# abowman6/CBET_RayTracing_3D

Hardware: AMD Instinct MI355X
Metric: ray-steps/sec, OMEGA 60-beam 256^3 sweep (higher is better)
Workload: dtype f64

## Files before the change

### cbet_raytracing_3d_amd/build.py

```python
import os
import shutil
import subprocess
import sys

PKG = os.path.dirname(os.path.abspath(__file__))
ROOT = os.path.dirname(PKG)
CSRC = os.path.join(PKG, "csrc")
LIB_DIR = os.path.join(PKG, "lib")
LIB_PATH = os.path.join(LIB_DIR, "libcbet_mi355x.so")
SOURCES = ["cbet_kernels.hip", "cbet_trace_window.hip", "cbet_trace_exit.hip", "cbet_trace_path.hip", "cbet_grid_kernels.hip", "cbet_lpi.hip", "cbet_sph_modes.hip",
           "cbet_target.hip", "cbet_mesh.hip", "cbet_mesh_deposit.hip", "cbet_params.cpp", "cbet_context.cpp", "cbet_tables_abi.cpp", "cbet_trace_abi.cpp", "cbet_gain_abi.cpp",
           "cbet_host.cpp", "cbet_output.cpp", "cbet_sph_host.cpp", "cbet_target_host.cpp", "cbet_mesh_host.cpp", "cbet_mesh_deposit_host.cpp",
           "cbet_exchange_host.cpp", "cbet_lpi_host.cpp"]
HEADERS = [os.path.join(CSRC, "cbet_device.h"), os.path.join(CSRC, "cbet_host_internal.h"), os.path.join(CSRC, "cbet_relocate.h"), os.path.join(CSRC, "cbet_trace_common.h"), os.path.join(CSRC, "cbet_trace_diag.h"), os.path.join(CSRC, "cbet_hd.h"), os.path.join(CSRC, "cbet_node_model.h"), os.path.join(CSRC, "cbet_node_kernel.h"), os.path.join(CSRC, "cbet_target_model.h"), os.path.join(CSRC, "cbet_mesh_model.h"), os.path.join(CSRC, "cbet_state_model.h"), os.path.join(CSRC, "cbet_mesh_deposit_model.h"), os.path.join(CSRC, "cbet_gain_model.h"), os.path.join(CSRC, "cbet_lpi_model.h"), os.path.join(ROOT, "include", "cbet_mi355x.h"),
           os.path.join(ROOT, "include", "cbet_omega_beams.h")]

FLAGS = ["-O3", "-std=c++17", "--offload-arch=gfx950", "-ffp-contract=off", "-fPIC", "-shared",
         "-Wall", "-Wextra", "-Wno-unused-result", "-mllvm", "-structurizecfg-skip-uniform-regions=true"]


def hipcc():
    exe = shutil.which("hipcc") or "/opt/rocm/bin/hipcc"
    if not os.path.exists(exe):
        raise RuntimeError("hipcc not found (need ROCm to build the gfx950 library)")
    return exe


def is_stale():
    if not os.path.exists(LIB_PATH):
        return True
    built = os.path.getmtime(LIB_PATH)
    deps = [os.path.join(CSRC, s) for s in SOURCES] + HEADERS + [os.path.abspath(__file__),
                                                                os.path.join(ROOT, "tools", "cbet_gpu.cpp"),
                                                                os.path.join(ROOT, "tools", "cbet_reference_shaped.cpp"),
                                                                os.path.join(ROOT, "include", "cbet_reference_api.hpp")]
    return any(os.path.getmtime(d) > built for d in deps)


def build(force=False, verbose=False, extra_flags=()):
    if not force and not is_stale():
        return LIB_PATH
    os.makedirs(LIB_DIR, exist_ok=True)
    cmd = [hipcc()] + FLAGS + list(extra_flags) + [
        "-I", os.path.join(ROOT, "include"), "-I", CSRC,
        "-o", LIB_PATH] + [os.path.join(CSRC, s) for s in SOURCES] + ["-lrccl"]
    if verbose:
        print(" ".join(cmd), flush=True)
    run = subprocess.run(cmd, stderr=subprocess.PIPE, text=True)
    sys.stderr.write(run.stderr)
    if run.returncode != 0 and "structurizecfg-skip-uniform-regions" in run.stderr:
        print("build: this hipcc does not know -structurizecfg-skip-uniform-regions; building without it", flush=True)
        k = cmd.index("-structurizecfg-skip-uniform-regions=true")
        subprocess.check_call(cmd[:k - 1] + cmd[k + 1:])
    elif run.returncode != 0:
        raise subprocess.CalledProcessError(run.returncode, cmd)
    build_cli(verbose)
    build_ref_shaped(verbose)
    return LIB_PATH


CLI_PATH = os.path.join(PKG, "lib", "cbet-gpu")


def build_cli(verbose=False):
    cmd = ["g++", "-O2", "-std=c++17", "-I", os.path.join(ROOT, "include"),
           os.path.join(ROOT, "tools", "cbet_gpu.cpp"), "-o", CLI_PATH,
           "-L", LIB_DIR, "-lcbet_mi355x", "-Wl,-rpath,$ORIGIN", "-Wl,-rpath-link," + "/opt/rocm/lib"]
    if verbose:
        print(" ".join(cmd), flush=True)
    subprocess.check_call(cmd)
    return CLI_PATH


REF_SHAPED_PATH = os.path.join(PKG, "lib", "cbet-ref-shaped")


def build_ref_shaped(verbose=False):
    cmd = [hipcc(), "-O2", "-std=c++17", "-I", os.path.join(ROOT, "include"),
           os.path.join(ROOT, "tools", "cbet_reference_shaped.cpp"), "-o", REF_SHAPED_PATH,
           "-L", LIB_DIR, "-lcbet_mi355x", "-Wl,-rpath,$ORIGIN"]
    if verbose:
        print(" ".join(cmd), flush=True)
    subprocess.check_call(cmd)
    return REF_SHAPED_PATH


def build_variant(name, extra_flags=(), verbose=False):
    out_dir = os.path.join(ROOT, "build_alt")
    os.makedirs(out_dir, exist_ok=True)
    out = os.path.join(out_dir, "libcbet_%s.so" % name)
    cmd = [hipcc()] + FLAGS + list(extra_flags) + ["-I", os.path.join(ROOT, "include"), "-I", CSRC, "-o", out] + \
        [os.path.join(CSRC, s) for s in SOURCES] + ["-lrccl"]
    if verbose:
        print(" ".join(cmd), flush=True)
    subprocess.check_call(cmd)
    return out


if __name__ == "__main__":
    if len(sys.argv) > 2 and sys.argv[1] == "--variant":
        print(build_variant(sys.argv[2], sys.argv[3:], verbose=True))
    else:
        print(build(force="--force" in sys.argv, verbose=True))
```

### cbet_raytracing_3d_amd/csrc/cbet_trace_window.hip

```cpp
#include <hip/hip_runtime.h>

#include <cstddef>
#include <type_traits>

#if defined(__HIP_DEVICE_COMPILE__) && !defined(__gfx950__)
#error "cbet_trace_window.hip is written for gfx950 (CDNA4) only"
#endif

#include "cbet_trace_common.h"
#include "cbet_trace_diag.h"

namespace cbet {
namespace {

#define CBET_BALLOT(cond) __builtin_amdgcn_ballot_w64(cond)
#define CBET_LANES(mask) __builtin_amdgcn_inverse_ballot_w64(mask)
#define CBET_USUAL(cond) __builtin_expect(!!(cond), 1)
#define CBET_RARE(cond) __builtin_expect(!!(cond), 0)
#define CBET_SELDOM(cond) __builtin_expect_with_probability(!!(cond), 0, 0.9)

template <int WX_, int WY_, int WZ_, bool PAD, bool XORSW = false>
struct Tile {
    static constexpr int WX = WX_, WY = WY_, WZ = WZ_;
    static constexpr int XM = WX - 1, YM = WY - 1, ZM = WZ - 1;
    static constexpr bool ROT = PAD && WZ == 16;
    static constexpr int YS = (PAD && !ROT) ? WZ + 1 : WZ;
    static constexpr int XS = (PAD && !ROT) ? WY * YS + 4 : WY * WZ;
    static constexpr bool XOR = ROT && XORSW;
    static __device__ __forceinline__ int zr(int tx, int ty, int tz)
    {
        return XOR ? (tz ^ ((tx & 3) << 2) ^ (ty << 1)) : (ROT ? ((tz + 7 * tx + 3 * ty) & ZM) : tz);
    }
    static_assert(!XOR || (WX == 8 && WY == 8 && WZ == 16), "the swizzle terms are written for the 8 x 8 x 16 box");
    static __device__ __forceinline__ int xterm(int tx) { return __mul24(tx, XS * 8 + 32) & ~0x80; }
    static __device__ __forceinline__ int yterm(int ty) { return __mul24(ty, YS * 8 + 16); }
    static constexpr int N = WX * XS;
    static constexpr int SX = WX - 2, SY = WY - 2, SZ = WZ - 2;
    static constexpr bool BRICK = WZ == 16 && WY == 8;
    static constexpr int DT = WX * WY * WZ;
    static __device__ __forceinline__ int slot_d(int tx, int ty, int tz) { return (tx * WY + ty) * WZ + tz; }
};

struct Origin {
    int x, y, z;
};

template <int M>
__device__ __forceinline__ int abs_in(int o, int r) { return o + ((r - o) & M); }

template <int C>
struct Corner {
    static constexpr int index = C;
    template <class V> static __device__ __forceinline__ V x(V v0, V v1) { return (C & 1) ? v1 : v0; }
    template <class V> static __device__ __forceinline__ V z(V v0, V v1) { return (C & 2) ? v1 : v0; }
    template <class V> static __device__ __forceinline__ V y(V v0, V v1) { return (C & 4) ? v1 : v0; }
};
template <class F>
__device__ __forceinline__ void each_corner(F f)
{
    f(Corner<0>{}); f(Corner<1>{}); f(Corner<2>{}); f(Corner<3>{}); f(Corner<4>{}); f(Corner<5>{}); f(Corner<6>{}); f(Corner<7>{});
}

struct WaveCounters {
    int n_atomics = 0;
    int n_miss = 0;
    unsigned steps_miss = 0;
    unsigned slabs_bsteps = 0;
    int pend = 0;
    [[no_unique_address]] WaveDiag dg;
};

template <bool W32>
struct Grid {
    double *p;
};
template <bool W32>
__device__ __forceinline__ void grid_add(const TraceArgs &a, Grid<W32> g, int node, double v)
{
    if constexpr (W32) global_add(a, reinterpret_cast<double *>(reinterpret_cast<char *>(g.p) + ((unsigned)node * 8u)), v);
    else global_add(a, &g.p[node], v);
}
template <bool W32>
__device__ __forceinline__ void grid_add_far(const TraceArgs &a, Grid<W32> g, long index, double v) { global_add(a, &g.p[index], v); }

template <class G>
__device__ __forceinline__ void write_back(const TraceArgs &a, double *tile, int slot, G edep, int node, double v, WaveCounters &wc)
{
    wc.pend += (CBET_BALLOT(v != 0.0) != 0ull) ? 1 : 0;
    if (v != 0.0) {
        tile[slot] = 0.0;
        ++wc.n_atomics;
        grid_add(a, edep, node, v);
    }
}
template <class G>
__device__ __forceinline__ void write_back_far(const TraceArgs &a, double *tile, int slot, G edep, long index, double v, WaveCounters &wc)
{
    wc.pend += (CBET_BALLOT(v != 0.0) != 0ull) ? 1 : 0;
    if (v != 0.0) {
        grid_add_far(a, edep, index, v);
        tile[slot] = 0.0;
        ++wc.n_atomics;
    }
}

template <class F>
__device__ __forceinline__ void miss_add8(unsigned long long hbm_m, WaveCounters &wc, F add8)
{
    if (CBET_RARE(hbm_m != 0ull)) {
        wc.pend += 8;
        if (CBET_LANES(hbm_m)) add8();
    }
}

template <class T, int AX, int COUNT, class G>
__device__ __forceinline__ void retire_planes(const TraceArgs &a, double *tile, const Origin &o, int coord, int step,
                                              int lane, G edep, int sXh, int sYh, WaveCounters &wc)
{
    constexpr int WO = AX == 0 ? T::WY : T::WX, OM = WO - 1;
    constexpr int IT = (WO * T::WZ + kWave - 1) / kWave;
    constexpr int RS = kWave / T::WZ;
    static_assert(IT == 1 || (IT == 2 && 2 * RS == WO), "a plane is one entry per lane, or two in the halves of the other axis");
    static_assert(!T::XOR || IT == 1 || (RS == 4 && T::YS == 16 && T::XS == 128), "the second entry's slot is written for the 8 x 8 x 16 box");
    constexpr int SLOT_X = AX == 0 ? (RS * T::YS) ^ ((2 * RS) & T::ZM) : RS * T::XS;
    const int r0 = lane / T::WZ, r1 = lane & T::ZM, k = abs_in<T::ZM>(o.z, r1);
    const int d0 = (r0 - (AX == 0 ? o.y : o.x)) & OM, dnode = ((d0 & RS) ? -RS : RS) * (AX == 0 ? sYh : sXh);
    const bool in_plane = !(WO * T::WZ < kWave) || lane < WO * T::WZ;
    double v[COUNT * IT];
    int slot[COUNT * IT], node[COUNT * IT];
#pragma unroll
    for (int pl = 0; pl < COUNT; ++pl) {
        const int c = coord + pl * step;
        const int fixed = c & (AX == 0 ? T::XM : T::YM);
#pragma unroll
        for (int e = 0; e < IT; ++e) {
            const int q = pl * IT + e, re = r0 + e * RS;
            if (e == 1 && T::XOR) {
                slot[q] = slot[q - 1] ^ SLOT_X;
                node[q] = node[q - 1] + dnode;
            } else if (AX == 0) {
                slot[q] = fixed * T::XS + re * T::YS + T::zr(fixed, re, r1);
                node[q] = c * sXh + __mul24(abs_in<T::YM>(o.y, re), sYh) + k;
            } else {
                slot[q] = re * T::XS + fixed * T::YS + T::zr(re, fixed, r1);
                node[q] = __mul24(abs_in<T::XM>(o.x, re), sXh) + c * sYh + k;
            }
            const bool ok = in_plane && CBET_AUDIT(a, (unsigned)slot[q] < (unsigned)T::N);
            v[q] = ok ? tile[slot[q]] : 0.0;
        }
    }
#pragma unroll
    for (int q = 0; q < COUNT * IT; ++q) write_back(a, tile, slot[q], edep, node[q], v[q], wc);
}

template <class T, int AX, int NC, class G>
__device__ __forceinline__ void retire_plane(const TraceArgs &a, double *tile, const Origin &o, int coord, int lane,
                                             G edep, int sXh, int sYh, WaveCounters &wc, int coff, long gstride)
{
    constexpr int WO = AX == 0 ? T::WY : T::WX;
    constexpr int IT = (WO * T::WZ + kWave - 1) / kWave;
    const int fixed = coord & (AX == 0 ? T::XM : T::YM);
#pragma unroll
    for (int e = 0; e < IT; ++e) {
        const int idx = e * kWave + lane;
        const bool in_plane = !(WO * T::WZ < kWave) || idx < WO * T::WZ;
        const int r0 = idx / T::WZ, r1 = idx & T::ZM;
        int slot, node, slot_d;
        const int k = abs_in<T::ZM>(o.z, r1);
        if (AX == 0) {
            slot = fixed * T::XS + r0 * T::YS + T::zr(fixed, r0, r1);
            slot_d = T::slot_d(fixed, r0, r1);
            node = coord * sXh + __mul24(abs_in<T::YM>(o.y, r0), sYh) + k;
        } else {
            slot = r0 * T::XS + fixed * T::YS + T::zr(r0, fixed, r1);
            slot_d = T::slot_d(r0, fixed, r1);
            node = __mul24(abs_in<T::XM>(o.x, r0), sXh) + coord * sYh + k;
        }
        const bool ok = in_plane && CBET_AUDIT(a, (unsigned)slot < (unsigned)T::N);
        const double v = ok ? tile[slot] : 0.0;
        if (NC > 1) {
#pragma unroll
            for (int q = 1; q < NC; ++q) {
                const int sq = coff + (q - 1) * T::DT + slot_d;
                write_back_far(a, tile, sq, edep, q * gstride + node, ok ? tile[sq] : 0.0, wc);
            }
        }
        write_back(a, tile, slot, edep, node, v, wc);
    }
}

template <class T, int NC, class G>
__device__ __forceinline__ void retire_zplane(const TraceArgs &a, double *tile, const Origin &o, int coord, int lane,
                                              G edep, int sXh, int sYh, WaveCounters &wc, int coff, long gstride)
{
    static_assert(T::WX * T::WY <= kWave, "one z-plane entry per lane");
    const int r0 = lane / T::WY, r1 = lane & T::YM, fixed = coord & T::ZM;
    const int slot = r0 * T::XS + r1 * T::YS + T::zr(r0, r1, fixed);
    const int node = __mul24(abs_in<T::XM>(o.x, r0), sXh) + __mul24(abs_in<T::YM>(o.y, r1), sYh) + coord;
    const bool ok = (!(T::WX * T::WY < kWave) || lane < T::WX * T::WY) && CBET_AUDIT(a, (unsigned)slot < (unsigned)T::N);
    const double v = ok ? tile[slot] : 0.0;
    if (NC > 1) {
        const int slot_d = T::slot_d(r0, r1, fixed);
#pragma unroll
        for (int q = 1; q < NC; ++q) {
            const int sq = coff + (q - 1) * T::DT + slot_d;
            write_back_far(a, tile, sq, edep, q * gstride + node, ok ? tile[sq] : 0.0, wc);
        }
    }
    write_back(a, tile, slot, edep, node, v, wc);
}

template <class T, class G>
__device__ __forceinline__ void retire_zbrick(const TraceArgs &a, double *tile, const Origin &o, int zb, int lane,
                                              G edep, int sXh, int sYh, WaveCounters &wc)
{
    static_assert(T::WY == 8 && T::WZ == 16, "a brick is 8 rows of 8 planes per tile x index");
    const int ty = lane >> 3, kz = lane & 7;
    const int tz = (zb + kz) & T::ZM;
    const int base_node = __mul24(abs_in<T::YM>(o.y, ty), sYh) + zb + kz;
    constexpr int ROUND = 4;
#pragma unroll
    for (int t0 = 0; t0 < T::WX; t0 += ROUND) {
        double v[ROUND];
        int slot[ROUND];
#pragma unroll
        for (int q = 0; q < ROUND; ++q) {
            slot[q] = (t0 + q) * T::XS + ty * T::YS + T::zr(t0 + q, ty, tz);
            v[q] = CBET_AUDIT(a, (unsigned)slot[q] < (unsigned)T::N) ? tile[slot[q]] : 0.0;
        }
#pragma unroll
        for (int q = 0; q < ROUND; ++q) write_back(a, tile, slot[q], edep, abs_in<T::XM>(o.x, t0 + q) * sXh + base_node, v[q], wc);
    }
}

template <class T, int NC, class G>
__device__ __forceinline__ void flush_box(const TraceArgs &a, double *tile, const Origin &o, int lane, G edep,
                                          int sXh, int sYh, WaveCounters &wc, int coff, long gstride)
{
    for (int t = 0; t < T::WX; ++t)
        retire_plane<T, 0, NC>(a, tile, o, o.x + t, lane, edep, sXh, sYh, wc, coff, gstride);
}

__device__ __forceinline__ int follow_plane_axis(int r, unsigned long long mm, int S)
{
    const unsigned long long edge = __builtin_amdgcn_ballot_w64((unsigned)(r - 1) >= (unsigned)(S - 1)) & mm;
    if (CBET_USUAL(edge == 0ull)) return 0;
    const unsigned long long hi = __builtin_amdgcn_ballot_w64(r >= S) & edge;
    const bool at_hi = hi != 0ull, at_lo = hi != edge;
    if (at_hi == at_lo) return 0;
    if (at_hi) {
        if ((__builtin_amdgcn_ballot_w64(r <= 1) & mm) != 0ull) return (__builtin_amdgcn_ballot_w64(r > S) & mm) != 0ull ? 1 : 0;
        return (S >= 6 && (__builtin_amdgcn_ballot_w64(r <= 2) & mm) == 0ull) ? 2 : 1;
    }
    if ((__builtin_amdgcn_ballot_w64(r >= S - 1) & mm) != 0ull) return (__builtin_amdgcn_ballot_w64(r < 0) & mm) != 0ull ? -1 : 0;
    return (S >= 6 && (__builtin_amdgcn_ballot_w64(r >= S - 2) & mm) == 0ull) ? -2 : -1;
}

__device__ __forceinline__ int follow_brick_axis(int r, unsigned long long mm)
{
    if ((__builtin_amdgcn_ballot_w64((unsigned)r > 14u) & mm) == 0ull) return 0;
    const bool below = (__builtin_amdgcn_ballot_w64(r < 0) & mm) != 0ull, above = (__builtin_amdgcn_ballot_w64(r > 14) & mm) != 0ull;
    const bool needs_lo = (__builtin_amdgcn_ballot_w64(r <= 7) & mm) != 0ull, needs_hi = (__builtin_amdgcn_ballot_w64(r >= 7) & mm) != 0ull;
    return (below && !needs_hi) ? -1 : ((above && !needs_lo) ? 1 : 0);
}

template <class T, int NC, class G>
__device__ __forceinline__ bool follow_box(const TraceArgs &a, double *tile, Origin &o, unsigned long long mm, int lx,
                                           int ly, int lz, int lane, G edep, int sXh, int sYh, WaveCounters &wc,
                                           int coff, long gstride)
{
    auto leave = [&](auto axis, int d, int lo, int hi) {
        constexpr int AX = decltype(axis)::value;
        const int first = d < 0 ? hi : lo, step = d < 0 ? -1 : 1, n = d < 0 ? -d : d;
        if constexpr (NC == 1) {
            if (n == 2) retire_planes<T, AX, 2>(a, tile, o, first, step, lane, edep, sXh, sYh, wc);
            else retire_planes<T, AX, 1>(a, tile, o, first, step, lane, edep, sXh, sYh, wc);
        } else {
            for (int q = 0; q < n; ++q) retire_plane<T, AX, NC>(a, tile, o, first + q * step, lane, edep, sXh, sYh, wc, coff, gstride);
        }
    };
    const int dx = follow_plane_axis(lx - o.x, mm, T::SX);
    const int dy = follow_plane_axis(ly - o.y, mm, T::SY);
    if (dx != 0) { wc.dg.retire_begin(); leave(std::integral_constant<int, 0>{}, dx, o.x, o.x + T::WX - 1); wc.dg.retire_end(); }
    o.x += dx;
    if (dy != 0) { wc.dg.retire_begin(); leave(std::integral_constant<int, 1>{}, dy, o.y, o.y + T::WY - 1); wc.dg.retire_end(); }
    o.y += dy;
    int dz;
    if constexpr (T::BRICK) {
        dz = 8 * follow_brick_axis(lz - o.z, mm);
        if (dz != 0) { wc.dg.retire_begin(); retire_zbrick<T>(a, tile, o, dz < 0 ? o.z + 8 : o.z, lane, edep, sXh, sYh, wc); wc.dg.retire_end(); }
    } else {
        dz = follow_plane_axis(lz - o.z, mm, T::SZ);
        if (dz != 0)
            retire_zplane<T, NC>(a, tile, o, dz < 0 ? o.z + T::WZ - 1 : o.z, lane, edep, sXh, sYh, wc, coff, gstride);
        for (int q = 1; q < (dz < 0 ? -dz : dz); ++q)
            retire_zplane<T, NC>(a, tile, o, dz < 0 ? o.z + T::WZ - 1 - q : o.z + q, lane, edep, sXh, sYh, wc, coff, gstride);
    }
    o.z += dz;
    const bool moved = (dx | dy | dz) != 0;
    wc.slabs_bsteps += moved ? (1u << 16) : 0u;
    return moved;
}

template <class T>
__device__ __forceinline__ bool holds(const Origin &o, int lx, int ly, int lz)
{
    return (unsigned)(lx - o.x) <= (unsigned)T::SX && (unsigned)(ly - o.y) <= (unsigned)T::SY &&
           (unsigned)(lz - o.z) <= (unsigned)T::SZ;
}

template <class T>
__device__ __forceinline__ int box_near_axes(const Origin &o, int nx, int ny, int nz)
{
    const int lo = kRelocateDeep + 1;
    const unsigned tx = (unsigned)((o.x - lo) | (nx - 3 - T::SX - o.x)), ty = (unsigned)((o.y - lo) | (ny - 3 - T::SY - o.y)),
                   tz = (unsigned)((o.z - lo) | (nz - 3 - T::SZ - o.z));
    return (int)((tx >> 31) | ((ty >> 31) << 1) | ((tz >> 31) << 2));
}

typedef double dbl2 __attribute__((ext_vector_type(2)));

template <bool WIDE>
__device__ __forceinline__ void record_issue(const StepRecord *base, unsigned cell, dbl2 &kxy, dbl2 &kzk)
{
    if constexpr (WIDE) {
        const char *p = reinterpret_cast<const char *>(base) + ((unsigned long long)cell << 5);
        asm volatile("global_load_dwordx4 %0, %2, off\n\tglobal_load_dwordx4 %1, %2, off offset:16\n\t; CBET_RECORD_ISSUE %0 %1"
                     : "=&v"(kxy), "=&v"(kzk)
                     : "v"(p)
                     : "memory");
    } else {
        const unsigned off = cell << 5;
        asm volatile("s_nop 4\n\tglobal_load_dwordx4 %0, %2, %3\n\tglobal_load_dwordx4 %1, %2, %3 offset:16\n\t; CBET_RECORD_ISSUE %0 %1"
                     : "=&v"(kxy), "=&v"(kzk)
                     : "v"(off), "s"(base)
                     : "memory");
    }
}

__device__ __forceinline__ void record_wait(dbl2 &kxy, dbl2 &kzk, int pend)
{
    asm volatile("; CBET_RECORD_WAIT %0 %1\n\t"
                 "s_cmp_eq_u32 %2, 0\n\t"
                 "s_cbranch_scc1 .Lrw_0_%=\n\t"
                 "s_cmp_ge_u32 %2, 8\n\t"
                 "s_cbranch_scc1 .Lrw_8_%=\n\t"
                 "s_cmp_ge_u32 %2, 4\n\t"
                 "s_cbranch_scc1 .Lrw_4_%=\n\t"
                 "s_cmp_ge_u32 %2, 2\n\t"
                 "s_cbranch_scc1 .Lrw_2_%=\n\t"
                 "s_waitcnt vmcnt(1)\n\t"
                 "s_branch .Lrw_end_%=\n"
                 ".Lrw_2_%=:\n\t"
                 "s_waitcnt vmcnt(2)\n\t"
                 "s_branch .Lrw_end_%=\n"
                 ".Lrw_4_%=:\n\t"
                 "s_waitcnt vmcnt(4)\n\t"
                 "s_branch .Lrw_end_%=\n"
                 ".Lrw_8_%=:\n\t"
                 "s_waitcnt vmcnt(8)\n\t"
                 "s_branch .Lrw_end_%=\n"
                 ".Lrw_0_%=:\n\t"
                 "s_waitcnt vmcnt(0)\n"
                 ".Lrw_end_%=:"
                 : "+v"(kxy), "+v"(kzk)
                 : "s"(pend)
                 : "memory", "scc");
}

__device__ __forceinline__ void record_wait_all(dbl2 &kxy, dbl2 &kzk)
{
    asm volatile("; CBET_RECORD_WAIT %0 %1\n\ts_waitcnt vmcnt(0)" : "+v"(kxy), "+v"(kzk) : : "memory");
}

__device__ __forceinline__ void exit_planes_load(dbl2 &bx, dbl2 &by, dbl2 &bz)
{
    const void *args = (const void *)__builtin_amdgcn_kernarg_segment_ptr();
    asm volatile("s_load_dwordx4 %0, %3, %4\n\ts_load_dwordx4 %1, %3, %5\n\ts_load_dwordx4 %2, %3, %6\n\ts_waitcnt lgkmcnt(0)"
                 : "=&s"(bx), "=&s"(by), "=&s"(bz)
                 : "s"(args), "i"(offsetof(TraceArgs, exit_planes)), "i"(offsetof(TraceArgs, exit_planes) + 16),
                   "i"(offsetof(TraceArgs, exit_planes) + 32));
}

__device__ __forceinline__ int add3(int a, int b, int c)
{
    int r;
    asm("v_add3_u32 %0, %1, %2, %3" : "=v"(r) : "v"(a), "v"(b), "v"(c));
    return r;
}

__device__ __forceinline__ int xad1(int f, int c)
{
    int r;
    asm("v_xad_u32 %0, %1, 1, %2" : "=v"(r) : "v"(f), "v"(c));
    return r;
}

__device__ __forceinline__ double max_abs3(double a, double b, double c)
{
    double r;
    asm("v_max_f64 %0, |%1|, |%2|" : "=v"(r) : "v"(a), "v"(b));
    asm("v_max_f64 %0, %1, |%2|" : "=v"(r) : "v"(r), "v"(c));
    return r;
}

__device__ __forceinline__ void commit(int &var, int value)
{
    asm volatile("s_mov_b32 %0, %1" : "+s"(var) : "s"(__builtin_amdgcn_readfirstlane(value)));
}
__device__ __forceinline__ void commit(unsigned long long &var, unsigned long long value)
{
    asm volatile("s_mov_b64 %0, %1" : "+s"(var) : "s"(value));
}
__device__ __forceinline__ void commit_v(int &var, int value) { asm volatile("v_mov_b32 %0, %1" : "+v"(var) : "v"(value)); }

__device__ __forceinline__ void cell_step(int &c, unsigned long long up, unsigned long long dn)
{
    asm("s_nop 1\n\tv_addc_co_u32_e64 %0, vcc, 0, %0, %1\n\tv_subbrev_co_u32_e64 %0, vcc, 0, %0, %2" : "+v"(c) : "s"(up), "s"(dn) : "vcc");
}
__device__ __forceinline__ void cell_step3(int &ci, int &cj, int &ck, unsigned long long upx, unsigned long long dnx,
                                           unsigned long long upy, unsigned long long dny, unsigned long long upz,
                                           unsigned long long dnz)
{
    asm("s_nop 1\n\t"
        "v_addc_co_u32_e64 %0, vcc, 0, %0, %3\n\tv_addc_co_u32_e64 %1, vcc, 0, %1, %5\n\tv_addc_co_u32_e64 %2, vcc, 0, %2, %7\n\t"
        "v_subbrev_co_u32_e64 %0, vcc, 0, %0, %4\n\tv_subbrev_co_u32_e64 %1, vcc, 0, %1, %6\n\tv_subbrev_co_u32_e64 %2, vcc, 0, %2, %8"
        : "+v"(ci), "+v"(cj), "+v"(ck)
        : "s"(upx), "s"(dnx), "s"(upy), "s"(dny), "s"(upz), "s"(dnz)
        : "vcc");
}

__device__ __forceinline__ int mad24(int a, int b, int c)
{
    int r;
    asm("s_nop 1\n\tv_mad_i32_i24 %0, %1, %2, %3" : "=v"(r) : "v"(a), "s"(b), "v"(c));
    return r;
}


#ifdef CBET_DEBUG_BOUNDS
constexpr bool kAudited = true;
#else
constexpr bool kAudited = false;
#endif
constexpr double kNearTol = 0.5001;
constexpr double kFarJump = 1.4998;

template <int WZ, bool GENERIC, int CBET, bool STATS>
__global__ void __launch_bounds__(kWave, (CBET == 4) ? 1 : 4) k_trace_window(const TraceArgs a)
{
    using T = Tile<8, 8, WZ, true, CBET == 0>;
    using TB = Tile<4, 8, 8, false>;
    constexpr bool IDX64 = GENERIC;
    constexpr int NC = (CBET == 4) ? 4 : 1;
    constexpr bool ACC = (CBET == 0);
    constexpr bool PIPE = ACC;
    constexpr int NSLOT = T::N + TB::N;
    constexpr int NLDS = NSLOT + (NC - 1) * T::DT;
    __shared__ double s_val[NLDS];
    const int lane = threadIdx.x;

    int beam, patch;
    if (!work_item(a, blockIdx.x, beam, patch)) return;
    const Grid<!IDX64> edep{a.edep + (long)(beam - a.grid_beam0) * a.grid_stride};
    const bool absorb = GENERIC ? (a.absorption == 1) : true;

    Ray s = {};
    int li;
    const bool launched = launch_lane(a, beam, patch, lane, s, li);
    unsigned long long live = __ballot(launched);
    if (live == 0ull) return;
    const int tot_rays = __popcll(live);

    const int nx = a.nx, ny = a.ny, nz = a.nz;
    const int sYh = a.sYh, sXh = a.sXh;
    unsigned cell = launched ? (unsigned)((s.ci * ny + s.cj) * nz + s.ck) : 0u;
    double fcx = (double)s.ci, fcy = (double)s.cj, fcz = (double)s.ck;
    int tot_steps = 0;
    WaveCounters wc;

    double *const tileA = s_val, *const tileB = s_val + T::N;
    Origin oA{0, 0, 0}, oB{0, 0, 0};
    unsigned long long hbm = 0ull;
    int b_active = 0;
    {
        const int src = ((live >> 27) & 1ull) ? 27 : (__ffsll((long long)live) - 1);
        for (int z = lane; z < NLDS; z += kWave) s_val[z] = 0.0;
        oA.x = __builtin_amdgcn_readlane(s.ci, src) + 1 - T::WX / 2;
        oA.y = __builtin_amdgcn_readlane(s.cj, src) + 1 - T::WY / 2;
        oA.z = __builtin_amdgcn_readlane(s.ck, src) + 1 - 4;
        if (T::BRICK) oA.z &= ~7;
        __syncthreads();
    }
    int near = 7;
    wc.dg.begin();

    dbl2 rec_kxy, rec_kzk;
    const StepRecord *rec_base = a.steprec;
    asm volatile("" : "+s"(rec_base));
    double dt = a.dt;
    auto gather_record = [&]() {
        unsigned c = CBET_LANES(live) ? cell : 0u;
        asm("" : "+v"(c));
#ifdef CBET_DEBUG_BOUNDS
        if (!(c < a.audit_nodes)) { audit_fail(a); c = 0u; }
#endif
        record_issue<IDX64>(rec_base, c, rec_kxy, rec_kzk);
        wc.pend = 0;
    };
    auto await_record = [&]() {
        wc.dg.wait_begin();
        if (CBET == 0 && !kAudited) record_wait(rec_kxy, rec_kzk, wc.pend);
        else record_wait_all(rec_kxy, rec_kzk);
        wc.dg.wait_end();
    };
    gather_record();
    await_record();
    const double *const gk = CBET && a.gain ? a.gain + (long)(beam - a.grid_beam0) * a.hsize : nullptr;
    double gained = 0.0;

    const bool flx = (lane & 1) != 0, fly = (lane & 2) != 0, flz = (lane & 8) != 0;
    const int pfx = flx ? 1 : 0, pfy = fly ? 1 : 0, pfz = flz ? 1 : 0;

    double q0 = 0.0, q1 = 0.0, q2 = 0.0, q3 = 0.0;

    int slow = 7;
    double Fx0 = 0, Fx1 = 0, Fy0 = 0, Fy1 = 0, Fz0 = 0, Fz1 = 0;
    int X0 = 0, X1 = 0, Y0 = 0, Y1 = 0, Z0 = 0, Z1 = 0;
    double inc = 0.0;
    int tile_off = 0;
    unsigned long long miss_m = 0ull;
    int own_slot = 0, own_node = 0;
    auto lds_add8 = [&](const double *w) {
        auto add = [&](int byte, double v) {
            if (CBET_AUDIT(a, (unsigned)byte < (unsigned)NSLOT * 8u))
                __hip_atomic_fetch_add(static_cast<double *>(__builtin_assume_aligned(reinterpret_cast<char *>(s_val) + byte, 8)),
                                       v, __ATOMIC_RELAXED, __HIP_MEMORY_SCOPE_WORKGROUP);
        };
        if constexpr (T::XOR) {
            int ax0, ax1, by0, by1, cz0, cz1;
            if (CBET_USUAL(b_active == 0)) {
                ax0 = T::xterm(X0 & T::XM); ax1 = T::xterm(X1 & T::XM);
                by0 = T::yterm(Y0 & T::YM); by1 = T::yterm(Y1 & T::YM);
                cz0 = (Z0 & T::ZM) << 3; cz1 = (Z1 & T::ZM) << 3;
            } else {
                const bool toB = tile_off != 0;
                const int xm = toB ? TB::XM : T::XM, zm = toB ? TB::ZM : T::ZM;
                const int xmul = toB ? TB::XS * 8 : T::XS * 8 + 32, ymul = toB ? TB::YS * 8 : T::YS * 8 + 16;
                const int keep = toB ? ~0 : ~0x80, off8 = tile_off * 8;
                static_assert(TB::YM == T::YM, "one y mask for both boxes");
                ax0 = (__mul24(X0 & xm, xmul) & keep) | off8; ax1 = (__mul24(X1 & xm, xmul) & keep) | off8;
                by0 = __mul24(Y0 & T::YM, ymul); by1 = __mul24(Y1 & T::YM, ymul);
                cz0 = (Z0 & zm) << 3; cz1 = (Z1 & zm) << 3;
            }
            auto at = [](int ax, int by, int cz) { return (int)__builtin_amdgcn_bitop3_b32(ax, by, cz, 0x96); };
            each_corner([=](auto c) { add(at(c.x(ax0, ax1), c.y(by0, by1), c.z(cz0, cz1)), w[c.index]); });
        } else {
            auto add8 = [&](int xm, int ym, int zm, int xs, int ys, int off, int rot) {
                const int xa = X0 & xm, xb = X1 & xm, ya = Y0 & ym, yb = Y1 & ym;
                const int x0 = __mul24(xa, xs * 8) + off * 8, x1 = __mul24(xb, xs * 8) + off * 8;
                const int y0 = __mul24(ya, ys * 8), y1 = __mul24(yb, ys * 8);
                const int ra = 7 * xa * rot, rb = 7 * xb * rot, sa = 3 * ya * rot, sb = 3 * yb * rot;
                auto zb = [&](int z, int r) { return ((z + r) & zm) * 8; };
                if constexpr (T::ROT) {
                    const int xy00 = x0 | y0, xy10 = x1 | y0, xy01 = x0 | y1, xy11 = x1 | y1, zm8 = zm * 8;
                    auto at = [&](int xy, int z, int r) { return (((z + r) * 8) & zm8) | xy; };
                    each_corner([&](auto c) {
                        add(at(c.y(c.x(xy00, xy10), c.x(xy01, xy11)), c.z(Z0, Z1), c.x(ra, rb) + c.y(sa, sb)), w[c.index]);
                    });
                } else {
                    each_corner([&](auto c) {
                        add(add3(c.x(x0, x1), c.y(y0, y1), zb(c.z(Z0, Z1), c.x(ra, rb) + c.y(sa, sb))), w[c.index]);
                    });
                }
            };
            if (b_active == 0) {
                add8(T::XM, T::YM, T::ZM, T::XS, T::YS, 0, T::ROT ? 1 : 0);
            } else {
                const bool toB = tile_off != 0;
                add8(toB ? TB::XM : T::XM, toB ? TB::YM : T::YM, toB ? TB::ZM : T::ZM, toB ? TB::XS : T::XS,
                     toB ? TB::YS : T::YS, tile_off, (T::ROT && !toB) ? 1 : 0);
            }
        }
    };
    auto hbm_add8 = [&](const double *w) {
        const int nX0 = __mul24(X0, sXh), nX1 = __mul24(X1, sXh), nY0 = __mul24(Y0, sYh), nY1 = __mul24(Y1, sYh);
        each_corner([&](auto c) { grid_add(a, edep, c.x(nX0, nX1) + c.y(nY0, nY1) + c.z(Z0, Z1), w[c.index]); });
        wc.n_atomics += 8;
    };

    auto deposit_step = [&](unsigned long long lds_m, unsigned long long hbm_m) {
        const double zi0 = Fz0 * inc, zi1 = Fz1 * inc;
        const double zy00 = zi0 * Fy0, zy10 = zi1 * Fy0, zy01 = zi0 * Fy1, zy11 = zi1 * Fy1;
        double wgt[8];
        wgt[0] = zy00 * Fx0;
        wgt[1] = zy00 * Fx1;
        wgt[2] = zy10 * Fx0;
        wgt[3] = zy10 * Fx1;
        wgt[4] = zy01 * Fx0;
        wgt[5] = zy01 * Fx1;
        wgt[6] = zy11 * Fx0;
        wgt[7] = zy11 * Fx1;
        if (CBET_LANES(lds_m)) lds_add8(wgt);
        miss_add8(hbm_m, wc, [&]() {
            hbm_add8(wgt);
            ++wc.n_miss;
        });
        if (CBET == 4) {
            const bool inbox = CBET_LANES(lds_m);
            if (inbox && tile_off == 0) {
                if (CBET_AUDIT(a, (unsigned)(own_slot + 2 * T::DT) < (unsigned)NLDS)) {
                    __hip_atomic_fetch_add(&s_val[own_slot], q1, __ATOMIC_RELAXED, __HIP_MEMORY_SCOPE_WORKGROUP);
                    __hip_atomic_fetch_add(&s_val[own_slot + T::DT], q2, __ATOMIC_RELAXED, __HIP_MEMORY_SCOPE_WORKGROUP);
                    __hip_atomic_fetch_add(&s_val[own_slot + 2 * T::DT], q3, __ATOMIC_RELAXED, __HIP_MEMORY_SCOPE_WORKGROUP);
                }
            } else if (inbox || CBET_LANES(hbm_m)) {
                grid_add_far(a, edep, a.comp_stride + own_node, q1);
                grid_add_far(a, edep, 2 * a.comp_stride + own_node, q2);
                grid_add_far(a, edep, 3 * a.comp_stride + own_node, q3);
                wc.n_atomics += 3;
            }
        }
    };

    double S[8] = {0, 0, 0, 0, 0, 0, 0, 0};
    unsigned long long restart_m = 0ull;
    bool p_odd = true;
    auto accumulate = [&]() {
        const double zi0 = Fz0 * inc, zi1 = Fz1 * inc;
        const double zy00 = zi0 * Fy0, zy10 = zi1 * Fy0, zy01 = zi0 * Fy1, zy11 = zi1 * Fy1;
        const double k = CBET_LANES(restart_m) ? 0.0 : 1.0;
        auto add = [&](double &sum, double w) { asm("v_fma_f64 %0, %0, %1, %2" : "+v"(sum) : "v"(k), "v"(w)); };
        add(S[0], zy00 * Fx0);
        add(S[1], zy00 * Fx1);
        add(S[2], zy10 * Fx0);
        add(S[3], zy10 * Fx1);
        add(S[4], zy01 * Fx0);
        add(S[5], zy01 * Fx1);
        add(S[6], zy11 * Fx0);
        add(S[7], zy11 * Fx1);
    };
    auto flush_sums = [&](unsigned long long lds_m, unsigned long long hbm_m) {
        if (CBET_LANES(lds_m)) lds_add8(S);
        miss_add8(hbm_m, wc, [&]() { hbm_add8(S); });
    };

    auto step_tail = [&](int &tt) {
    asm volatile("" : "+v"(Fx0), "+v"(Fx1), "+v"(Fy0), "+v"(Fy1), "+v"(Fz0), "+v"(Fz1));
    await_record();
    if (absorb) {
        inc = rec_kzk.y * s.uray;
        s.uray -= inc;
    } else {
        inc = s.uray;
    }
    if (CBET >= 2) inc = q0;
    if constexpr (ACC && !PIPE) accumulate();
    unsigned long long died = CBET_BALLOT(s.uray <= s.ustop);
    const int faces = slow | near;
    if (CBET_RARE(faces != 0)) {
        dbl2 bx, by, bz;
        exit_planes_load(bx, by, bz);
        if (faces & 1) died |= CBET_BALLOT(s.px < bx.x) | CBET_BALLOT(s.px > bx.y);
        if (faces & 2) died |= CBET_BALLOT(s.py < by.x) | CBET_BALLOT(s.py > by.y);
        if (faces & 4) died |= CBET_BALLOT(s.pz < bz.x) | CBET_BALLOT(s.pz > bz.y);
    }
    died &= live;
    if (CBET_SELDOM(died != 0ull)) {
        asm volatile("");
        commit(tot_steps, tot_steps + __popcll(died) * (tt + 1));
        if constexpr (PIPE) {
            accumulate();
            asm volatile("v_mov_b64 %0, 0" : "+v"(inc));
            commit(restart_m, 0ull);
        }
        if constexpr (ACC) flush_sums(died & ~miss_m, died & miss_m);
        else deposit_step(died & ~miss_m, died & miss_m);
        commit(live, live & ~died);
        commit(hbm, hbm & live);
        commit(miss_m, miss_m & live);
        if (live == 0ull) commit(tt, a.nt - 1);
    }
    __builtin_amdgcn_wave_barrier();
    };

    for (int tt = 0; tt < a.nt; ++tt) {
        if constexpr (STATS || WaveDiag::kCountsWaveSteps) wc.steps_miss += 1u << 16;
        wc.dg.step_begin(near);
        s.vx -= rec_kxy.x;
        s.vy -= rec_kxy.y;
        s.vz -= rec_kzk.x;
        asm volatile("" : "+s"(dt));
        s.px += s.vx * dt;
        s.py += s.vy * dt;
        s.pz += s.vz * dt;
        const double fx = (s.px - a.xmin) * a.inv_dx;
        const double fy = (s.py - a.ymin) * a.inv_dy;
        const double fz = (s.pz - a.zmin) * a.inv_dz;
        const double g0x = fx - fcx, g0y = fy - fcy, g0z = fz - fcz;
        const unsigned long long upx = CBET_BALLOT(g0x >= kNearTol), dnx = CBET_BALLOT(g0x < kNearTol - 1.0),
                                 upy = CBET_BALLOT(g0y >= kNearTol), dny = CBET_BALLOT(g0y < kNearTol - 1.0),
                                 upz = CBET_BALLOT(g0z >= kNearTol), dnz = CBET_BALLOT(g0z < kNearTol - 1.0);
        slow = ((CBET_BALLOT(!(max_abs3(g0x, g0y, g0z) < kFarJump)) & live) != 0ull) ? 7 : near;
        if (CBET_USUAL(slow == 0)) {
            cell_step3(s.ci, s.cj, s.ck, upx, dnx, upy, dny, upz, dnz);
        } else {
            if (slow & 1) s.ci = relocate_closed(s.ci, fx, nx);
            else cell_step(s.ci, upx, dnx);
            if (slow & 2) s.cj = relocate_closed(s.cj, fy, ny);
            else cell_step(s.cj, upy, dny);
            if (slow & 4) s.ck = relocate_closed(s.ck, fz, nz);
            else cell_step(s.ck, upz, dnz);
        }
        const unsigned new_cell = (unsigned)mad24(mad24(s.ci, ny, s.cj), nz, s.ck);
        unsigned long long moved_m = 0ull;
        if constexpr (ACC) moved_m = CBET_BALLOT(new_cell != cell);
        cell = new_cell;
        gather_record();
        wc.dg.chain_end();
        asm volatile("" : "+v"(s.ci), "+v"(s.cj), "+v"(s.ck), "+v"(inc));
        fcx = (double)s.ci;
        fcy = (double)s.cj;
        fcz = (double)s.ck;
        if constexpr (!ACC) deposit_step(live & ~miss_m, miss_m);
        if constexpr (PIPE) accumulate();
        const double ox = (fx - fcx) - 0.5, oy = (fy - fcy) - 0.5, oz = (fz - fcz) - 0.5;
        const bool ngx = ox < 0, ngy = oy < 0, ngz = oz < 0;
        const bool all_negative = (live & ~(CBET_BALLOT(ngx) & CBET_BALLOT(ngy) & CBET_BALLOT(ngz))) == 0ull;
        if constexpr (ACC) {
            const unsigned long long fl_m = (all_negative && !p_odd) ? (live & moved_m) : live;
            if (CBET_USUAL(fl_m != 0ull)) {
                if (CBET_USUAL(miss_m == 0ull)) flush_sums(fl_m, 0ull);
                else flush_sums(fl_m & ~miss_m, fl_m & miss_m);
            }
            restart_m = fl_m;
            p_odd = !all_negative;
        }
        factor_pair(ox, pfx, Fx0, Fx1);
        factor_pair(oy, pfy, Fy0, Fy1);
        factor_pair(oz, pfz, Fz0, Fz1);
        int rx, ry, rz;
        if (CBET_USUAL(all_negative)) {
            rx = s.ci - oA.x;
            ry = s.cj - oA.y;
            rz = s.ck - oA.z;
            asm("" : "+v"(rx), "+v"(ry), "+v"(rz));
            X0 = xad1(pfx, s.ci); X1 = s.ci + pfx;
            Y0 = xad1(pfy, s.cj); Y1 = s.cj + pfy;
            Z0 = xad1(pfz, s.ck); Z1 = s.ck + pfz;
        } else {
            const int lx = s.ci + 1 - (ngx ? 1 : 0);
            const int ly = s.cj + 1 - (ngy ? 1 : 0);
            const int lz = s.ck + 1 - (ngz ? 1 : 0);
            rx = lx - oA.x;
            ry = ly - oA.y;
            rz = lz - oA.z;
            const bool hx = ngx != flx, hy = ngy != fly, hz = ngz != flz;
            X0 = lx + (hx ? 1 : 0); X1 = lx + (hx ? 0 : 1);
            Y0 = ly + (hy ? 1 : 0); Y1 = ly + (hy ? 0 : 1);
            Z0 = lz + (hz ? 1 : 0); Z1 = lz + (hz ? 0 : 1);
        }
        if (CBET && CBET_LANES(live)) {
            double ds = 0.0;
            if (gk || CBET >= 2) ds = sqrt_speed(__builtin_fma(s.vz, s.vz, __builtin_fma(s.vy, s.vy, s.vx * s.vx))) * a.dt;
            double u_eff = s.uray;
            if (gk) {
                const double x = gain_exponent<IDX64>(a, gk, X0, X1, Y0, Y1, Z0, Z1, Fx0, Fx1, Fy0, Fy1, Fz0, Fz1, sXh, sYh, ds);
                const double phi = gain_phi(x, (CBET_BALLOT(!(fabs(x) < kPhiSmallBelow)) & live) == 0ull);
                const double dg = s.uray * (x * phi);
                u_eff = s.uray * phi;
                gained += dg;
                s.uray = s.uray + dg;
            }
            if (CBET == 2) q0 = u_eff * ds;
            if (CBET == 4) {
                q0 = u_eff * ds;
                q1 = u_eff * (s.vx * a.dt);
                q2 = u_eff * (s.vy * a.dt);
                q3 = u_eff * (s.vz * a.dt);
                const int hi = s.ci + 1, hj = s.cj + 1, hk = s.ck + 1;
                own_slot = T::slot_d(hi & T::XM, hj & T::YM, hk & T::ZM) + NSLOT;
                own_node = __mul24(hi, sXh) + __mul24(hj, sYh) + hk;
            }
        }
        const unsigned long long memA = live & ~hbm;
        unsigned long long out_core = memA & ~(CBET_BALLOT((unsigned)rx <= (unsigned)T::SX) & CBET_BALLOT((unsigned)ry <= (unsigned)T::SY) &
                                               CBET_BALLOT((unsigned)rz <= (unsigned)T::SZ));
        if (CBET_RARE(b_active != 0)) {
            asm volatile("");
            if constexpr (STATS) wc.slabs_bsteps += 1u;
            const int abx = oA.x - oB.x, aby = oA.y - oB.y, abz = oA.z - oB.z;
            out_core |= hbm & ~(CBET_BALLOT((unsigned)(rx + abx) <= (unsigned)TB::SX) &
                                CBET_BALLOT((unsigned)(ry + aby) <= (unsigned)TB::SY) &
                                CBET_BALLOT((unsigned)(rz + abz) <= (unsigned)TB::SZ));
            tile_off = CBET_LANES(hbm) ? T::N : 0;
        }
        out_core |= miss_m;
        if (CBET_RARE(out_core != 0ull)) {
            wc.dg.arm_begin();
            const bool alive = CBET_LANES(live);
            int lx = rx + oA.x, ly = ry + oA.y, lz = rz + oA.z;
            asm volatile("" : "+v"(lx), "+v"(ly), "+v"(lz));
            Origin nA = oA, nB = oB;
            unsigned long long n_hbm = hbm, n_miss = 0ull;
            int n_bact = b_active, n_near, n_toff = tile_off;
            follow_box<T, NC>(a, tileA, nA, memA, lx, ly, lz, lane, edep, sXh, sYh, wc, NSLOT, a.comp_stride);
            const unsigned long long lost_mask =
                memA & ~(CBET_BALLOT((unsigned)(lx - nA.x) <= (unsigned)T::SX) & CBET_BALLOT((unsigned)(ly - nA.y) <= (unsigned)T::SY) &
                         CBET_BALLOT((unsigned)(lz - nA.z) <= (unsigned)T::SZ));
            if (CBET_USUAL(lost_mask == 0ull && n_bact == 0)) {
                n_near = box_near_axes<T>(nA, nx, ny, nz);
            } else {
                bool homeB = CBET_LANES(hbm);
                const bool inA = alive && holds<T>(nA, lx, ly, lz);
                const bool lost = alive && !homeB && !inA;
                if (n_bact != 0) {
                    follow_box<TB, 1>(a, tileB, nB, hbm, lx, ly, lz, lane, edep, sXh, sYh, wc, 0, 0);
                } else if (lost_mask != 0ull) {
                    const int src = __ffsll((long long)lost_mask) - 1;
                    const int sx = __builtin_amdgcn_readlane(lx, src), sy = __builtin_amdgcn_readlane(ly, src),
                              sz = __builtin_amdgcn_readlane(lz, src);
                    nB.x = sx - (TB::WX / 2 - 1);
                    nB.y = sy - (TB::WY / 2 - 1);
                    nB.z = sz - TB::SZ / 2;
                    n_bact = 1;
                }
                const bool inB = alive && holds<TB>(nB, lx, ly, lz);
                homeB = homeB || (lost && inB);
                if (alive && homeB && !inB && inA) homeB = false;
                n_hbm = CBET_BALLOT(alive && homeB);
                if (n_hbm == 0ull) {
                    __builtin_amdgcn_wave_barrier();
                    flush_box<TB, 1>(a, tileB, nB, lane, edep, sXh, sYh, wc, 0, 0);
                    n_bact = 0;
                }
                __builtin_amdgcn_wave_barrier();
                const bool useB = alive && homeB && inB;
                n_toff = useB ? T::N : 0;
                n_miss = live & ~CBET_BALLOT(useB || (alive && !homeB && inA));
                if constexpr (STATS) {
                    if (n_miss != 0ull) wc.steps_miss += 1u;
                    if (ACC && CBET_LANES(n_miss)) ++wc.n_miss;
                }
                n_near = n_miss != 0ull ? 7 : (box_near_axes<T>(nA, nx, ny, nz) | (n_bact == 0 ? 0 : box_near_axes<TB>(nB, nx, ny, nz)));
            }
            commit(oA.x, nA.x); commit(oA.y, nA.y); commit(oA.z, nA.z);
            commit(oB.x, nB.x); commit(oB.y, nB.y); commit(oB.z, nB.z);
            commit(hbm, n_hbm); commit(miss_m, n_miss);
            commit(b_active, n_bact); commit(near, n_near);
            commit_v(tile_off, n_toff);
            wc.pend = __builtin_amdgcn_readfirstlane(wc.pend);
            wc.dg.arm_end();
        } else if (CBET_RARE(near != 0)) {
            commit(near, box_near_axes<T>(oA, nx, ny, nz) | (b_active == 0 ? 0 : box_near_axes<TB>(oB, nx, ny, nz)));
        }
        step_tail(tt);
    }
    tot_steps += __popcll(live) * a.nt;

    if constexpr (PIPE) accumulate();
    if constexpr (ACC) flush_sums(live & ~miss_m, live & miss_m);
    else deposit_step(live & ~miss_m, live & miss_m);
    __syncthreads();
    flush_box<T, NC>(a, tileA, oA, lane, edep, sXh, sYh, wc, NSLOT, a.comp_stride);
    if (b_active != 0) flush_box<TB, 1>(a, tileB, oB, lane, edep, sXh, sYh, wc, 0, 0);

    if (CBET && a.beam_gain) {
        double t = gained;
#pragma unroll
        for (int off = 32; off > 0; off >>= 1) t += __shfl_xor(t, off, kWave);
        if (lane == 0 && t != 0.0) atomicAdd(&a.beam_gain[beam], t);
    }
    if (wc.dg.report(a, lane, tot_steps, tot_rays, wc.steps_miss >> 16)) return;
    if constexpr (STATS) {
        const int tot_at = wave_sum(wc.n_atomics), tot_miss = wave_sum(wc.n_miss);
        if (lane == 0) {
            atomicAdd(&a.counters[kCntGlobalAtomics], (unsigned long long)tot_at);
            atomicAdd(&a.counters[kCntEvictions], (unsigned long long)tot_miss);
            atomicAdd(&a.counters[kCntWaveSteps], (unsigned long long)(wc.steps_miss >> 16));
            atomicAdd(&a.counters[kCntWaveStepsMiss], (unsigned long long)(wc.steps_miss & 0xFFFFu));
            atomicAdd(&a.counters[kCntWaveStepsWide], (unsigned long long)(wc.slabs_bsteps & 0xFFFFu));
            atomicAdd(&a.counters[kCntSlabsRetired], (unsigned long long)(wc.slabs_bsteps >> 16));
        }
    }
    if (lane == 0) {
        atomicAdd(&a.counters[kCntSteps], (unsigned long long)tot_steps);
        atomicAdd(&a.counters[kCntRays], (unsigned long long)tot_rays);
    }
}

}

hipError_t launch_trace_window(const TraceArgs &a, bool force_idx64, hipStream_t stream)
{
    const long waves = a.item_count;
    if (waves <= 0) return hipSuccess;
    const dim3 grid((unsigned)waves), block(kWave);
    const unsigned long long grid_bytes = 8ull * (unsigned long long)a.sXh * (unsigned long long)(a.nx + 2);
    const bool generic = force_idx64 || (a.gain && 8ull * (unsigned long long)a.hsize >= (1ull << 32)) || a.absorption != 1 ||
                         grid_bytes >= (1ull << 32) ||
                         sizeof(StepRecord) * (unsigned long long)a.nx * a.ny * a.nz > (1ull << 32);
    auto go = [&](auto wz, auto cbet) {
        constexpr int WZ = decltype(wz)::value, CB = decltype(cbet)::value;
        if (a.stats) {
            if (generic) hipLaunchKernelGGL((k_trace_window<WZ, true, CB, true>), grid, block, 0, stream, a);
            else hipLaunchKernelGGL((k_trace_window<WZ, false, CB, true>), grid, block, 0, stream, a);
        } else {
            if (generic) hipLaunchKernelGGL((k_trace_window<WZ, true, CB, false>), grid, block, 0, stream, a);
            else hipLaunchKernelGGL((k_trace_window<WZ, false, CB, false>), grid, block, 0, stream, a);
        }
    };
    using std::integral_constant;
    if (a.quantity == 1) go(integral_constant<int, 8>{}, integral_constant<int, 4>{});
    else if (a.quantity == 2) go(integral_constant<int, 16>{}, integral_constant<int, 2>{});
    else if (a.gain || a.beam_gain) go(integral_constant<int, 16>{}, integral_constant<int, 1>{});
    else go(integral_constant<int, 16>{}, integral_constant<int, 0>{});
    return hipGetLastError();
}

}
```

Baseline: 174.9 billion.

## Keep shared-face corner sums for single-axis stray lanes instead of flushing to HBM

For lanes that miss the LDS tiles and move by one cell along exactly one axis, the accumulated 8-corner sums are partially kept: the four corners shared with the next cell are shifted over and carried forward, and only the four leaving corners are atomically added to global memory. This aims to halve global atomics on the miss path. The change also narrows the 'near' edge checks for miss lanes to per-axis ballots rather than forcing all axes, and derives the tile-B selection from the hbm mask instead of a per-lane tile offset. It adds ballot and branch overhead on the miss path and more complex accounting of pending atomics.

```diff
diff --git a/cbet_raytracing_3d_amd/build.py b/cbet_raytracing_3d_amd/build.py
--- a/cbet_raytracing_3d_amd/build.py
+++ b/cbet_raytracing_3d_amd/build.py
@@ -12,7 +12,7 @@
            "cbet_target.hip", "cbet_mesh.hip", "cbet_mesh_deposit.hip", "cbet_params.cpp", "cbet_context.cpp", "cbet_tables_abi.cpp", "cbet_trace_abi.cpp", "cbet_gain_abi.cpp",
            "cbet_host.cpp", "cbet_output.cpp", "cbet_sph_host.cpp", "cbet_target_host.cpp", "cbet_mesh_host.cpp", "cbet_mesh_deposit_host.cpp",
            "cbet_exchange_host.cpp", "cbet_lpi_host.cpp"]
-HEADERS = [os.path.join(CSRC, "cbet_device.h"), os.path.join(CSRC, "cbet_host_internal.h"), os.path.join(CSRC, "cbet_relocate.h"), os.path.join(CSRC, "cbet_trace_common.h"), os.path.join(CSRC, "cbet_trace_diag.h"), os.path.join(CSRC, "cbet_hd.h"), os.path.join(CSRC, "cbet_node_model.h"), os.path.join(CSRC, "cbet_node_kernel.h"), os.path.join(CSRC, "cbet_target_model.h"), os.path.join(CSRC, "cbet_mesh_model.h"), os.path.join(CSRC, "cbet_state_model.h"), os.path.join(CSRC, "cbet_mesh_deposit_model.h"), os.path.join(CSRC, "cbet_gain_model.h"), os.path.join(CSRC, "cbet_lpi_model.h"), os.path.join(ROOT, "include", "cbet_mi355x.h"),
+HEADERS = [os.path.join(CSRC, "cbet_device.h"), os.path.join(CSRC, "cbet_host_internal.h"), os.path.join(CSRC, "cbet_relocate.h"), os.path.join(CSRC, "cbet_stray.h"), os.path.join(CSRC, "cbet_trace_common.h"), os.path.join(CSRC, "cbet_trace_diag.h"), os.path.join(CSRC, "cbet_hd.h"), os.path.join(CSRC, "cbet_node_model.h"), os.path.join(CSRC, "cbet_node_kernel.h"), os.path.join(CSRC, "cbet_target_model.h"), os.path.join(CSRC, "cbet_mesh_model.h"), os.path.join(CSRC, "cbet_state_model.h"), os.path.join(CSRC, "cbet_mesh_deposit_model.h"), os.path.join(CSRC, "cbet_gain_model.h"), os.path.join(CSRC, "cbet_lpi_model.h"), os.path.join(ROOT, "include", "cbet_mi355x.h"),
            os.path.join(ROOT, "include", "cbet_omega_beams.h")]
 
 FLAGS = ["-O3", "-std=c++17", "--offload-arch=gfx950", "-ffp-contract=off", "-fPIC", "-shared",
diff --git a/cbet_raytracing_3d_amd/csrc/cbet_stray.h b/cbet_raytracing_3d_amd/csrc/cbet_stray.h
--- /dev/null
+++ b/cbet_raytracing_3d_amd/csrc/cbet_stray.h
@@ -0,0 +1,57 @@
+#ifndef CBET_STRAY_H_
+#define CBET_STRAY_H_
+
+#include "cbet_hd.h"
+
+namespace cbet {
+
+constexpr int kCornerX = 1, kCornerZ = 2, kCornerY = 4;
+constexpr bool stray_corner_on(int c, int bit, int leave) { return ((c & bit) != 0) == (leave != 0); }
+
+template <class M>
+struct StrayAxis {
+    M leave0, leave1;
+};
+
+template <class M>
+CBET_HD StrayAxis<M> stray_axis(M single, M flip, M down)
+{
+    const M stay1 = flip ^ down;
+    return {single & stay1, single & ~stay1};
+}
+
+template <class M>
+struct StrayPlan {
+    StrayAxis<M> x, y, z;
+    CBET_HD M kept() const { return x.leave0 | x.leave1 | y.leave0 | y.leave1 | z.leave0 | z.leave1; }
+    CBET_HD M stays(int c) const
+    {
+        return ((c & kCornerX) ? x.leave0 : x.leave1) | ((c & kCornerY) ? y.leave0 : y.leave1) | ((c & kCornerZ) ? z.leave0 : z.leave1);
+    }
+    CBET_HD M full(M lanes) const { return lanes & ~kept(); }
+    CBET_HD int issued(M lanes) const
+    {
+        auto some = [&](M m) { return (lanes & m) != 0 ? 1 : 0; };
+        return 8 * (full(lanes) != 0 ? 1 : 0) +
+               4 * (some(x.leave0) + some(x.leave1) + some(y.leave0) + some(y.leave1) + some(z.leave0) + some(z.leave1));
+    }
+};
+
+template <int BIT, int LEAVE, class V>
+CBET_HD void stray_keep_side(V (&S)[8])
+{
+    for (int c = 0; c < 8; ++c) {
+        if (!stray_corner_on(c, BIT, LEAVE)) continue;
+        S[c] = S[c ^ BIT];
+        S[c ^ BIT] = V(0);
+    }
+}
+template <int BIT, class V>
+CBET_HD void stray_keep_axis(V (&S)[8], bool leave0, bool leave1)
+{
+    if (leave0) stray_keep_side<BIT, 0>(S);
+    if (leave1) stray_keep_side<BIT, 1>(S);
+}
+
+}
+#endif
diff --git a/cbet_raytracing_3d_amd/csrc/cbet_trace_window.hip b/cbet_raytracing_3d_amd/csrc/cbet_trace_window.hip
--- a/cbet_raytracing_3d_amd/csrc/cbet_trace_window.hip
+++ b/cbet_raytracing_3d_amd/csrc/cbet_trace_window.hip
@@ -7,6 +7,7 @@
 #error "cbet_trace_window.hip is written for gfx950 (CDNA4) only"
 #endif
 
+#include "cbet_stray.h"
 #include "cbet_trace_common.h"
 #include "cbet_trace_diag.h"
 
@@ -104,12 +105,12 @@
     }
 }
 
-template <class F>
-__device__ __forceinline__ void miss_add8(unsigned long long hbm_m, WaveCounters &wc, F add8)
+template <class F, class GUARDED = std::true_type>
+__device__ __forceinline__ void miss_add8(unsigned long long hbm_m, WaveCounters &wc, F add8, int issued = 8, GUARDED = GUARDED())
 {
     if (CBET_RARE(hbm_m != 0ull)) {
-        wc.pend += 8;
-        if (CBET_LANES(hbm_m)) add8();
+        wc.pend += issued;
+        if (!GUARDED::value || CBET_LANES(hbm_m)) add8();
     }
 }
 
@@ -544,10 +545,10 @@
                 by0 = T::yterm(Y0 & T::YM); by1 = T::yterm(Y1 & T::YM);
                 cz0 = (Z0 & T::ZM) << 3; cz1 = (Z1 & T::ZM) << 3;
             } else {
-                const bool toB = tile_off != 0;
+                const bool toB = CBET_LANES(hbm);
                 const int xm = toB ? TB::XM : T::XM, zm = toB ? TB::ZM : T::ZM;
                 const int xmul = toB ? TB::XS * 8 : T::XS * 8 + 32, ymul = toB ? TB::YS * 8 : T::YS * 8 + 16;
-                const int keep = toB ? ~0 : ~0x80, off8 = tile_off * 8;
+                const int keep = toB ? ~0 : ~0x80, off8 = toB ? T::N * 8 : 0;
                 static_assert(TB::YM == T::YM, "one y mask for both boxes");
                 ax0 = (__mul24(X0 & xm, xmul) & keep) | off8; ax1 = (__mul24(X1 & xm, xmul) & keep) | off8;
                 by0 = __mul24(Y0 & T::YM, ymul); by1 = __mul24(Y1 & T::YM, ymul);
@@ -583,10 +584,34 @@
             }
         }
     };
-    auto hbm_add8 = [&](const double *w) {
+    typedef StrayPlan<unsigned long long> Strays;
+    auto hbm_add8 = [&](const double *w, unsigned long long hbm_m = 0ull, const Strays &sp = Strays()) {
         const int nX0 = __mul24(X0, sXh), nX1 = __mul24(X1, sXh), nY0 = __mul24(Y0, sYh), nY1 = __mul24(Y1, sYh);
-        each_corner([&](auto c) { grid_add(a, edep, c.x(nX0, nX1) + c.y(nY0, nY1) + c.z(Z0, Z1), w[c.index]); });
-        wc.n_atomics += 8;
+        auto add = [&](auto c) { grid_add(a, edep, c.x(nX0, nX1) + c.y(nY0, nY1) + c.z(Z0, Z1), w[c.index]); };
+        const unsigned long long kept = ACC ? sp.kept() : 0ull;
+        if (!ACC || CBET_LANES(hbm_m & ~kept)) {
+            each_corner(add);
+            wc.n_atomics += 8;
+        }
+        if (CBET_RARE(kept != 0ull)) {
+            auto side = [&](unsigned long long m, auto bit, auto leave) {
+                if (m != 0ull) {
+                    if (CBET_LANES(m)) {
+                        each_corner([&](auto c) {
+                            if constexpr (stray_corner_on(c.index, bit.value, leave.value)) add(c);
+                        });
+                        wc.n_atomics += 4;
+                    }
+                }
+            };
+            using std::integral_constant;
+            side(sp.x.leave0, integral_constant<int, kCornerX>{}, integral_constant<int, 0>{});
+            side(sp.x.leave1, integral_constant<int, kCornerX>{}, integral_constant<int, 1>{});
+            side(sp.y.leave0, integral_constant<int, kCornerY>{}, integral_constant<int, 0>{});
+            side(sp.y.leave1, integral_constant<int, kCornerY>{}, integral_constant<int, 1>{});
+            side(sp.z.leave0, integral_constant<int, kCornerZ>{}, integral_constant<int, 0>{});
+            side(sp.z.leave1, integral_constant<int, kCornerZ>{}, integral_constant<int, 1>{});
+        }
     };
 
     auto deposit_step = [&](unsigned long long lds_m, unsigned long long hbm_m) {
@@ -640,9 +665,42 @@
         add(S[6], zy11 * Fx0);
         add(S[7], zy11 * Fx1);
     };
-    auto flush_sums = [&](unsigned long long lds_m, unsigned long long hbm_m) {
+    auto flush_sums = [&](unsigned long long lds_m, unsigned long long hbm_m, const Strays &sp = Strays()) {
         if (CBET_LANES(lds_m)) lds_add8(S);
-        miss_add8(hbm_m, wc, [&]() { hbm_add8(S); });
+        miss_add8(hbm_m, wc, [&]() { hbm_add8(S, hbm_m, sp); }, __builtin_amdgcn_readfirstlane(sp.issued(hbm_m)), std::false_type{});
+    };
+    auto stray_plan = [&](unsigned long long lanes) {
+        unsigned long long far = 0ull;
+        auto axis = [&](int c, int pf, int n1, unsigned long long &moved, unsigned long long &down) {
+            const int d = c + pf - n1;
+            moved = CBET_BALLOT(d != 0);
+            down = CBET_BALLOT(d < 0);
+            far |= CBET_BALLOT((unsigned)(d + 1) > 2u);
+        };
+        unsigned long long mx, my, mz, dnx, dny, dnz;
+        axis(s.ci, pfx, X1, mx, dnx);
+        axis(s.cj, pfy, Y1, my, dny);
+        axis(s.ck, pfz, Z1, mz, dnz);
+        const unsigned long long one = lanes & ~far & (mx ^ my ^ mz) & ~(mx & my & mz);
+        constexpr unsigned long long kFlipX = 0xAAAAAAAAAAAAAAAAull, kFlipY = 0xCCCCCCCCCCCCCCCCull, kFlipZ = 0xFF00FF00FF00FF00ull;
+        return Strays{stray_axis(one & mx, kFlipX, dnx), stray_axis(one & my, kFlipY, dny), stray_axis(one & mz, kFlipZ, dnz)};
+    };
+    auto stray_keep = [&](const Strays &sp) {
+        auto side = [&](unsigned long long m, auto bit, auto leave) {
+            if (m != 0ull) {
+                if (CBET_LANES(m)) {
+                    asm volatile("");
+                    stray_keep_side<decltype(bit)::value, decltype(leave)::value>(S);
+                }
+            }
+        };
+        using std::integral_constant;
+        side(sp.x.leave0, integral_constant<int, kCornerX>{}, integral_constant<int, 0>{});
+        side(sp.x.leave1, integral_constant<int, kCornerX>{}, integral_constant<int, 1>{});
+        side(sp.y.leave0, integral_constant<int, kCornerY>{}, integral_constant<int, 0>{});
+        side(sp.y.leave1, integral_constant<int, kCornerY>{}, integral_constant<int, 1>{});
+        side(sp.z.leave0, integral_constant<int, kCornerZ>{}, integral_constant<int, 0>{});
+        side(sp.z.leave1, integral_constant<int, kCornerZ>{}, integral_constant<int, 1>{});
     };
 
     auto step_tail = [&](int &tt) {
@@ -729,11 +787,22 @@
         const bool all_negative = (live & ~(CBET_BALLOT(ngx) & CBET_BALLOT(ngy) & CBET_BALLOT(ngz))) == 0ull;
         if constexpr (ACC) {
             const unsigned long long fl_m = (all_negative && !p_odd) ? (live & moved_m) : live;
+            restart_m = fl_m;
             if (CBET_USUAL(fl_m != 0ull)) {
-                if (CBET_USUAL(miss_m == 0ull)) flush_sums(fl_m, 0ull);
-                else flush_sums(fl_m & ~miss_m, fl_m & miss_m);
+                if (CBET_USUAL(miss_m == 0ull)) {
+                    flush_sums(fl_m, 0ull);
+                } else if (all_negative && !p_odd) {
+                    const Strays sp = stray_plan(fl_m & miss_m);
+                    const unsigned long long kept = sp.kept();
+                    flush_sums(fl_m & ~miss_m, fl_m & miss_m, sp);
+                    if (kept != 0ull) {
+                        stray_keep(sp);
+                        restart_m = fl_m & ~kept;
+                    }
+                } else {
+                    flush_sums(fl_m & ~miss_m, fl_m & miss_m);
+                }
             }
-            restart_m = fl_m;
             p_odd = !all_negative;
         }
         factor_pair(ox, pfx, Fx0, Fx1);
@@ -842,13 +911,23 @@
                     if (n_miss != 0ull) wc.steps_miss += 1u;
                     if (ACC && CBET_LANES(n_miss)) ++wc.n_miss;
                 }
-                n_near = n_miss != 0ull ? 7 : (box_near_axes<T>(nA, nx, ny, nz) | (n_bact == 0 ? 0 : box_near_axes<TB>(nB, nx, ny, nz)));
+                if constexpr (ACC) {
+                    n_near = box_near_axes<T>(nA, nx, ny, nz) | (n_bact == 0 ? 0 : box_near_axes<TB>(nB, nx, ny, nz));
+                    if (n_miss != 0ull) {
+                        const int lo = kRelocateDeep + 1;
+                        n_near |= ((CBET_BALLOT(lx < lo) | CBET_BALLOT(lx > nx - 3)) & n_miss) != 0ull ? 1 : 0;
+                        n_near |= ((CBET_BALLOT(ly < lo) | CBET_BALLOT(ly > ny - 3)) & n_miss) != 0ull ? 2 : 0;
+                        n_near |= ((CBET_BALLOT(lz < lo) | CBET_BALLOT(lz > nz - 3)) & n_miss) != 0ull ? 4 : 0;
+                    }
+                } else {
+                    n_near = n_miss != 0ull ? 7 : (box_near_axes<T>(nA, nx, ny, nz) | (n_bact == 0 ? 0 : box_near_axes<TB>(nB, nx, ny, nz)));
+                }
             }
             commit(oA.x, nA.x); commit(oA.y, nA.y); commit(oA.z, nA.z);
             commit(oB.x, nB.x); commit(oB.y, nB.y); commit(oB.z, nB.z);
             commit(hbm, n_hbm); commit(miss_m, n_miss);
             commit(b_active, n_bact); commit(near, n_near);
-            commit_v(tile_off, n_toff);
+            if constexpr (!T::XOR) commit_v(tile_off, n_toff);
             wc.pend = __builtin_amdgcn_readfirstlane(wc.pend);
             wc.dg.arm_end();
         } else if (CBET_RARE(near != 0)) {
```

Result: no change. 174.8 billion (-0.1%).
